# MaxMax2016/MixGAN-TTS

Hardware: AMD Instinct MI355X
Metric: denoiser steps/sec (80-mel, L=1000 frames, B=16 per GPU) (higher is better)
Workload: dtype f32

## Files before the change

mixgan-tts_amd/csrc/denoiser_common.h:

```cpp
#pragma once
#include "conv_mfma.h"
#include <cstdlib>

int mg_device_cus();
unsigned *mg_host_err_device_ptr();
unsigned mg_persist_spin_limit();
static inline bool den_persist_allowed(int NL, int tiles_per_b, int chain_cap)
{
    const char *pe = std::getenv("MG_DENOISER_PERSIST");
    return !(pe && pe[0] == '0') && NL >= 3 && tiles_per_b <= chain_cap;
}

enum DpSyncWord {
    DP_SYNC_TICKET = 0,
    DP_SYNC_ERROR = 1,
    DP_SYNC_LAUNCHES = 2,
    DP_SYNC_DONE = 3,
    DP_SYNC_TICKET_B = 16,
    DP_SYNC_WORDS = 64
};
static_assert(DP_SYNC_TICKET_B < DP_SYNC_WORDS, "every counter word lies inside the reserved block");
static_assert((int)DP_SYNC_TICKET == MG_STATUS_TICKET && (int)DP_SYNC_ERROR == MG_STATUS_ERROR && (int)DP_SYNC_LAUNCHES == MG_STATUS_LAUNCHES &&
              (int)DP_SYNC_DONE == MG_STATUS_DONE && MG_STATUS_DONE + 1 == MG_STATUS_WORDS, "one contiguous copy");

struct DenLayout {
    size_t freq, in_w, in_b, mlp0, mlp2, skip_w, skip_b, out_w, out_b, layers, layer_stride;
    size_t l_wc, l_w3, l_wo, l_bc, l_b3, l_bo, l_wd, l_wp;
    size_t bw, in_wT, skip_wT, out_wT, wc_allT, blayers, blayer_stride;
    size_t bl_w3T, bl_woT;
    size_t slayers, slayer_stride, sl_wc, sl_w3, sl_wo;
    size_t in_w16, skip_w16, out_w16, p16layers, p16layer_stride, p_wc, p_w3, p_wo;
    size_t wc_all, bc_all;
    size_t jobs;
    size_t total;
};

static inline DenLayout den_layout(const mg_denoiser_dims *d, int flags)
{
    const int with_backward = flags & MG_DEN_BACKWARD;
    const int C = d->channels, H = d->cond_channels, M = d->mel_bins, NL = d->n_layers;
    DenLayout o;
    size_t p = 0;
    auto take = [&](size_t n) {
        size_t at = p;
        p += mg_align_up(n, 64);
        return at;
    };
    o.freq = take(C / 2);
    o.in_w = take(mg_conv_packed_floats(C, M, 1, MG_PACK_PLAIN));
    o.in_b = take(C);
    o.mlp0 = take((size_t)4 * C * C);
    o.mlp2 = take((size_t)4 * C * C);
    o.skip_w = take(mg_conv_packed_floats(C, C, 1, MG_PACK_PLAIN));
    o.skip_b = take(C);
    o.out_w = take(mg_conv_packed_floats(M, C, 1, MG_PACK_PLAIN));
    o.out_b = take(M);
    o.layers = p;
    size_t q = 0;
    auto ltake = [&](size_t n) {
        size_t at = q;
        q += mg_align_up(n, 64);
        return at;
    };
    o.l_wc = ltake(mg_conv_packed_floats(C, H, 1, MG_PACK_PLAIN));
    o.l_w3 = ltake(mg_conv_packed_floats(2 * C, C, 3, MG_PACK_GATE));
    o.l_wo = ltake(mg_conv_packed_floats(2 * C, C, 1, MG_PACK_PLAIN));
    o.l_bc = ltake(C);
    o.l_b3 = ltake(2 * C);
    o.l_bo = ltake(2 * C);
    o.l_wd = ltake((size_t)C * C);
    o.l_wp = ltake(d->multi_speaker ? (size_t)C * H : 0);
    o.layer_stride = q;
    p += q * NL;
    o.bw = p;
    o.in_wT = o.skip_wT = o.out_wT = o.wc_allT = o.blayers = o.blayer_stride = o.bl_w3T = o.bl_woT = 0;
    if (with_backward) {
        o.in_wT = take(mg_conv_packed_floats(C, M, 1, MG_PACK_DGRAD));
        o.skip_wT = take(mg_conv_packed_floats(C, C, 1, MG_PACK_DGRAD));
        o.out_wT = take(mg_conv_packed_floats(M, C, 1, MG_PACK_DGRAD));
        o.wc_allT = take((size_t)mg_conv_mblocks(H) * ((size_t)NL * C / 8) * 256);
        o.blayers = p;
        size_t r = 0;
        auto btake = [&](size_t n) {
            size_t at = r;
            r += mg_align_up(n, 64);
            return at;
        };
        o.bl_w3T = btake(mg_conv_packed_floats(2 * C, C, 3, MG_PACK_DGRAD));
        o.bl_woT = btake(mg_conv_packed_floats(2 * C, C, 1, MG_PACK_DGRAD));
        o.blayer_stride = r;
        p += r * NL;
    }
    o.slayers = o.slayer_stride = o.sl_wc = o.sl_w3 = o.sl_wo = 0;
    if (flags & MG_DEN_SPLIT) {
        o.slayers = p;
        size_t r = 0;
        auto stake = [&](size_t n) {
            size_t at = r;
            r += mg_align_up(n, 64);
            return at;
        };
        o.sl_wc = stake((size_t)(C / 32) * (H / 16) * 512);
        o.sl_w3 = stake((size_t)(2 * C / 32) * (3 * C / 16) * 512);
        o.sl_wo = stake((size_t)(2 * C / 32) * (C / 16) * 512);
        o.slayer_stride = r;
        p += r * NL;
    }
    o.in_w16 = o.skip_w16 = o.out_w16 = o.p16layers = o.p16layer_stride = o.p_wc = o.p_w3 = o.p_wo = 0;
    o.wc_all = o.bc_all = 0;
    if (flags & MG_DEN_P16) {
        o.in_w16 = take(mg_conv_packed_floats(C, M, 1, MG_PACK_PLAIN16));
        o.skip_w16 = take(mg_conv_packed_floats(C, C, 1, MG_PACK_PLAIN16));
        o.out_w16 = take(mg_conv_packed_floats(M, C, 1, MG_PACK_PLAIN16));
        o.p16layers = p;
        size_t r = 0;
        auto ptake = [&](size_t n) {
            size_t at = r;
            r += mg_align_up(n, 64);
            return at;
        };
        o.p_wc = ptake(mg_conv_packed_floats(C, H, 1, MG_PACK_PLAIN16));
        o.p_w3 = ptake(mg_conv_packed_floats(2 * C, C, 3, MG_PACK_GATE16));
        o.p_wo = ptake(mg_conv_packed_floats(2 * C, C, 1, MG_PACK_PLAIN16));
        o.p16layer_stride = r;
        p += r * NL;
        o.wc_all = take((size_t)NL * mg_conv_packed_floats(C, H, 1, MG_PACK_PLAIN));
        o.bc_all = take((size_t)NL * C);
    }
    p = mg_align_up(p, 64);
    o.jobs = p;
    p += 768 * 96 / 4;
    o.total = p;
    return o;
}

static inline int den_check(const mg_denoiser_dims *d)
{
    if (!d) return MG_ERR_ARG;
    if (d->n_layers <= 0 || d->n_layers > 256 || d->channels <= 0 || d->channels % 64 || d->cond_channels <= 0 ||
        d->cond_channels % 32 || d->mel_bins <= 0)
        return MG_ERR_SHAPE;
    return MG_OK;
}

struct DenWs {
    size_t emb, h1pre, h1, s, dvec, hvec, x, skip, y, x0, h, g, sig, tnh, conds, total;
    size_t act_stride;
    size_t sync, gran;
    size_t team;
};

static inline size_t den_persist_tiles(int B, int L) { return (size_t)B * ((L + 15) / 16); }

static inline DenWs den_ws(const mg_denoiser_dims *d, int B, int L, int save)
{
    const size_t C = d->channels, NL = d->n_layers;
    const size_t act = mg_align_up((size_t)B * C * L, 64);
    DenWs w;
    size_t p = 0;
    auto take = [&](size_t n) {
        size_t at = p;
        p += mg_align_up(n, 64);
        return at;
    };
    w.emb = take(B * C);
    w.h1pre = take(B * 4 * C);
    w.h1 = take(B * 4 * C);
    w.s = take(B * C);
    w.dvec = take(NL * B * C);
    w.hvec = d->multi_speaker ? take(NL * B * C) : w.dvec;
    w.x = take(act);
    w.skip = take(act);
    w.y = take(act);
    w.x0 = save ? take(act) : w.x;
    w.act_stride = save ? act : 0;
    const size_t nact = save ? NL : 1;
    w.h = take(act * nact);
    w.g = take(act * nact);
    w.sig = save ? take(act * nact) : 0;
    w.tnh = save ? take(act * nact) : 0;
    w.conds = take(act);
    w.sync = take(DP_SYNC_WORDS);
    w.gran = take(2 * den_persist_tiles(B, L) * 2 * C * 2);
    w.team = take(den_persist_tiles(B, L) <= 128 && C == 256 ? 2 * den_persist_tiles(B, L) * 256 * (18 + 16) * 2 : 0);
    w.total = p;
    return w;
}

struct DenBws {
    size_t dout, dz_all, dx_all, dh_all, dy, dx0, scratch, dd_all, dhv_all, ds, dm, da, btop, bbot, total;
    size_t sync, gran;
};

static inline DenBws den_bws(const mg_denoiser_dims *d, int B, int L)
{
    const size_t C = d->channels, NL = d->n_layers, H = d->cond_channels, M = d->mel_bins;
    const size_t act = mg_align_up((size_t)B * C * L, 64);
    DenBws w;
    size_t p = 0;
    auto take = [&](size_t n) {
        size_t at = p;
        p += mg_align_up(n, 64);
        return at;
    };
    w.dout = take(2 * act);
    w.dz_all = take(2 * NL * act);
    w.dx_all = take((NL + 1) * act);
    w.dh_all = take(NL * act);
    w.dy = take(act);
    w.dx0 = take(act);
    size_t sc = 0;
    const int c = (int)C, h = (int)H, m = (int)M, nl = (int)NL;
    const int shapes[6][3] = {{2 * c, c, 3}, {2 * c, c, 1}, {nl * c, h, 1}, {c, m, 1}, {c, c, 1}, {m, c, 1}};
    for (const auto &sh : shapes) {
        const size_t need = mg_conv1d_wgrad_scratch_floats(sh[0], sh[1], sh[2]);
        if (need > sc) sc = need;
    }
    {
        const size_t g3 = mg_conv1d_wgrad_grouped_scratch_floats(2 * c, c, 3, nl);
        const size_t go = mg_conv1d_wgrad_grouped_scratch_floats(c, c, 1, nl);
        if (g3 > sc) sc = g3;
        if (go > sc) sc = go;
    }
    w.scratch = take(sc);
    w.btop = take((size_t)NL * C);
    w.bbot = take(C);
    w.dd_all = take(NL * B * C);
    w.dhv_all = take(NL * B * C);
    w.ds = take(B * C);
    w.dm = take(B * 4 * C);
    w.da = take(B * 4 * C);
    w.sync = take(DP_SYNC_WORDS);
    w.gran = take(2 * den_persist_tiles(B, L) * 2 * (2 * C) * 2);
    w.total = p;
    return w;
}

static __global__ void step_embed_kernel(const int64_t *__restrict__ t, const float *__restrict__ freq,
                                  float *__restrict__ emb, int B, int C)
{
    const int half = C / 2;
    const int idx = blockIdx.x * blockDim.x + threadIdx.x;
    if (idx >= B * half) return;
    const int b = idx / half, i = idx - b * half;
    const double ang = (double)((float)t[b] * freq[i]);
    emb[(size_t)b * C + i] = (float)sin(ang);
    emb[(size_t)b * C + half + i] = (float)cos(ang);
}

__device__ __forceinline__ float mg_softplus(float v) { return v > 20.f ? v : log1pf(expf(v)); }

template <int BC>
__global__ __launch_bounds__(256) void small_linear_kernel(const float *__restrict__ W, long w_zs,
                                                           const float *__restrict__ in, float *__restrict__ out,
                                                           long out_zs, const float *__restrict__ add, long add_zs,
                                                           float *__restrict__ pre, int B, int N, int K, int mish,
                                                           int in_rows)
{
    const int lane = threadIdx.x & 63;
    const int j = blockIdx.x * 4 + (threadIdx.x >> 6);
    const int b0 = blockIdx.y * BC;
    const int z = blockIdx.z;
    if (j >= N) return;
    const float *w = W + (size_t)z * w_zs + (size_t)j * K;
    float acc[BC];
#pragma unroll
    for (int b = 0; b < BC; ++b) acc[b] = 0.f;
    if ((K & 255) == 0) {
        for (int i = lane * 4; i < K; i += 256) {
            const f32x4 wv = *reinterpret_cast<const f32x4 *>(w + i);
            f32x4 xv[BC];
#pragma unroll
            for (int b = 0; b < BC; ++b)
                xv[b] = *reinterpret_cast<const f32x4 *>(in + (size_t)(min(b0 + b, B - 1) % in_rows) * K + i);
#pragma unroll
            for (int b = 0; b < BC; ++b) {
                float t = acc[b];
                t = fmaf(wv[0], xv[b][0], t);
                t = fmaf(wv[1], xv[b][1], t);
                t = fmaf(wv[2], xv[b][2], t);
                t = fmaf(wv[3], xv[b][3], t);
                acc[b] = t;
            }
        }
    } else {
        for (int i = lane; i < K; i += 64) {
            const float wv = w[i];
#pragma unroll
            for (int b = 0; b < BC; ++b)
                if (b0 + b < B) acc[b] = fmaf(wv, in[(size_t)((b0 + b) % in_rows) * K + i], acc[b]);
        }
    }
#pragma unroll
    for (int b = 0; b < BC; ++b) {
        float v = acc[b];
#pragma unroll
        for (int o = 32; o > 0; o >>= 1) v += __shfl_xor(v, o, 64);
        if (lane == 0 && b0 + b < B) {
            if (pre) pre[(size_t)(b0 + b) * N + j] = v;
            if (mish) v = v * tanhf(mg_softplus(v));
            const size_t o = (size_t)z * out_zs + (size_t)(b0 + b) * N + j;
            if (add) v += add[(size_t)z * add_zs + (size_t)(b0 + b) * N + j];
            out[o] = v;
        }
    }
}

static inline int small_linear(const float *W, long w_zs, const float *in, float *out, long out_zs, const float *add,
                               long add_zs, float *pre, int B, int N, int K, int Z, int mish, hipStream_t st,
                               int in_rows = 0)
{
    constexpr int BC = 8;
    dim3 grid(mg_cdiv(N, 4), mg_cdiv(B, BC), Z);
    hipLaunchKernelGGL(small_linear_kernel<BC>, grid, dim3(256), 0, st, W, w_zs, in, out, out_zs, add, add_zs, pre, B, N,
                       K, mish, in_rows > 0 ? in_rows : B);
    MG_LAUNCH_CHECK();
    return MG_OK;
}

static __global__ void small_outer_kernel(const float *__restrict__ a, long a_zs, long a_bs, const float *__restrict__ c,
                                   float *__restrict__ out, int Z, int B, int N, int K)
{
    const size_t n = (size_t)Z * N * K;
    for (size_t idx = (size_t)blockIdx.x * blockDim.x + threadIdx.x; idx < n; idx += (size_t)gridDim.x * blockDim.x) {
        const int j = (int)(idx % K);
        const int i = (int)((idx / K) % N);
        const int z = (int)(idx / ((size_t)K * N));
        float s = 0.f;
        for (int b = 0; b < B; ++b) s = fmaf(a[(size_t)z * a_zs + (size_t)b * a_bs + i], c[(size_t)b * K + j], s);
        out[idx] = s;
    }
}

static __global__ __launch_bounds__(256) void small_linear_t_kernel(const float *__restrict__ W, long w_zs,
                                                                    const float *__restrict__ a, long a_zs, long a_bs,
                                                                    float *__restrict__ out, int Z, int B, int N, int K)
{
    __shared__ float red[4][64];
    const int lane = threadIdx.x & 63, wave = threadIdx.x >> 6;
    const int j = blockIdx.x * 64 + lane;
    const int b = blockIdx.y, z = blockIdx.z;
    const float *w = W + (size_t)z * w_zs + min(j, K - 1);
    const float *av = a + (size_t)z * a_zs + (size_t)b * a_bs;
    const int per = (N + 3) / 4;
    const int i0 = wave * per, i1 = min(N, i0 + per);
    float s = 0.f;
#pragma unroll 8
    for (int i = i0; i < i1; ++i) s = fmaf(w[(size_t)i * K], av[i], s);
    red[wave][lane] = s;
    __syncthreads();
    if (wave == 0 && j < K) {
        const float t = red[0][lane] + red[1][lane] + red[2][lane] + red[3][lane];
        if (Z > 1) atomicAdd(out + (size_t)b * K + j, t);
        else out[(size_t)b * K + j] = t;
    }
}

static __global__ void mish_bwd_kernel(const float *__restrict__ dm, const float *__restrict__ x, float *__restrict__ da, int n)
{
    const int i = blockIdx.x * blockDim.x + threadIdx.x;
    if (i >= n) return;
    const float v = x[i];
    const float ts = tanhf(mg_softplus(v));
    const float sg = 1.f / (1.f + expf(-v));
    da[i] = dm[i] * (ts + v * (1.f - ts * ts) * sg);
}

static __global__ void scale_mask_kernel(const float *__restrict__ in, long in_bs, const float *__restrict__ mask,
                                  float *__restrict__ out, float alpha, int CL, size_t n)
{
    for (size_t i = (size_t)blockIdx.x * blockDim.x + threadIdx.x; i < n; i += (size_t)gridDim.x * blockDim.x) {
        const size_t b = i / CL;
        const size_t r = i - b * CL;
        out[i] = mask[i] > 0.f ? alpha * in[b * in_bs + r] : 0.f;
    }
}
```

mixgan-tts_amd/csrc/denoiser_persist.h:

```cpp
#pragma once
#include "common.h"
#include "denoiser_common.h"
#include "resblock_fused.h"

#define DP_SPIN_LIMIT (1u << 21)
#define DP_F_ROLES 1
#define DP_F_WITHHOLD 2

typedef unsigned long long dp_u64;
typedef __attribute__((address_space(1))) dp_u64 dp_gu64;
typedef __attribute__((address_space(1))) unsigned dp_gu32;
typedef __attribute__((address_space(1))) const char dp_gcchar;
typedef __attribute__((address_space(1))) const f32x4 dp_gcf32x4;

struct PersistArgs {
    const float *x_t;
    const float *cond;
    const float *cproj;
    float *cproj_out;
    const float *in_w, *in_b;
    const float *layers;
    size_t layer_stride, l_wc, l_w3, l_wo, l_bc, l_b3, l_bo;
    const float *p16layers;
    size_t p16layer_stride, p_wc, p_w3, p_wo;
    const float *skip_w, *skip_b, *out_w, *out_b;
    const float *hvec, *dvec;
    int vec_rows;
    float *out;
    const int64_t *t;
    const float *coef1, *coef2, *logvar;
    const float *noise;
    unsigned long long seed;
    unsigned long long noise_stream;
    float *x0_out;
    dp_u64 *gran;
    dp_u64 *team;
    unsigned *sync;
    unsigned *host_err;
    unsigned spin_limit;
    float *x0_save, *y_save, *skip_save;
    float *h_save, *g_save, *sig_save, *tnh_save;
    size_t act_stride;
    unsigned long long *dbg;
    int dbg_wave;
    int B, L, M, NL, tiles_per_b, post, clip, n_steps;
    int flags;
    float rsNL;
    int b_split;
    const float *x_t2, *hvec2, *dvec2, *cond2;
    float *out2;
};

struct DpIterK1 {
    static constexpr int N = 8, KW = 1;
    static __device__ __forceinline__ int chunk(int it) { return it; }
    static __device__ __forceinline__ int tap(int) { return 0; }
};
struct DpIterHead {
    static constexpr int N = 3, KW = 1;
    static __device__ __forceinline__ int chunk(int it) { return it; }
    static __device__ __forceinline__ int tap(int) { return 0; }
};
struct DpIterCentre {
    static constexpr int N = 8, KW = 3;
    static __device__ __forceinline__ int chunk(int it) { return it; }
    static __device__ __forceinline__ int tap(int) { return 1; }
};
struct DpIterOuter {
    static constexpr int N = 16, KW = 3;
    static __device__ __forceinline__ int chunk(int it) { return it >> 1; }
    static __device__ __forceinline__ int tap(int it) { return (it & 1) * 2; }
};

__device__ __forceinline__ int dp_pos(int ch) { return ((ch & 1) << 2) | ((ch >> 1) & 3); }
template <int NTC>
__device__ __forceinline__ int dp_at(int ch, int col) { return (((ch >> 3) * NTC + col) << 3) + dp_pos(ch); }

#ifndef DP_DIST_BIG
#define DP_DIST_BIG 3
#endif
template <int NMB, int NNB, int NTC, class IT, int DIST, bool SBASE>
__device__ __forceinline__ void dp_mfma_loop_at(f32x16 (&acc)[NMB][NNB], const f32x4 *const (&ap)[NMB], unsigned loff,
                                                const float *__restrict__ tile)
{
    static_assert(DIST >= 1 && DIST <= 3, "ring of 4 slots");
    f32x4 ring[4][NMB];
    f32x4 bb[2][NNB];
    dp_gcchar *ub[NMB];
    if (SBASE) {
#pragma unroll
        for (int i = 0; i < NMB; ++i) {
            const unsigned long long v = reinterpret_cast<unsigned long long>(ap[i]);
            const unsigned lo = __builtin_amdgcn_readfirstlane((unsigned)v), hi = __builtin_amdgcn_readfirstlane((unsigned)(v >> 32));
            ub[i] = (dp_gcchar *)(((unsigned long long)hi << 32) | lo);
        }
    }
    auto sbase = [&](int i, int qb) {
        dp_gcchar *p = ub[i] + (size_t)qb * 1024;
        asm volatile("" : "+s"(p));
        return p;
    };
    if (SBASE) asm volatile("" : "+v"(loff));
    auto wload = [&](int i, int qb, int d) -> f32x4 {
        if (SBASE) return *(dp_gcf32x4 *)(ub[i] + (size_t)qb * 1024 + loff + d * 1024);
        return ap[i][(size_t)(qb + d) * 64];
    };
    auto qbase = [](int it) { return (IT::chunk(it) * IT::KW + IT::tap(it)) * 4; };
    auto boff = [](int it) { return IT::chunk(it) * (4 * NTC * 8) + IT::tap(it) * 8; };
    {
        const int q0 = qbase(0);
#pragma unroll
        for (int s = 0; s < DIST; ++s)
#pragma unroll
            for (int i = 0; i < NMB; ++i) ring[s][i] = wload(i, q0, s);
        const float *T0 = tile + boff(0);
#pragma unroll
        for (int j = 0; j < NNB; ++j) bb[0][j] = *reinterpret_cast<const f32x4 *>(T0 + 32 * 8 * j);
    }
#pragma unroll 1
    for (int it = 0; it < IT::N; ++it) {
        const int itn = it + 1 < IT::N ? it + 1 : IT::N - 1;
        const int qc = qbase(it), qn = qbase(itn);
        const float *Tc = tile + boff(it), *Tn = tile + boff(itn);
        dp_gcchar *bc[NMB], *bn[NMB];
        if (SBASE) {
            asm volatile("" : "+v"(loff));
#pragma unroll
            for (int i = 0; i < NMB; ++i) {
                bc[i] = sbase(i, qc);
                bn[i] = sbase(i, qn);
            }
        }
#pragma unroll
        for (int u = 0; u < 4; ++u) {
#pragma unroll
            for (int i = 0; i < NMB; ++i) {
                constexpr int LIM = 4 - DIST;
                const int d = u < LIM ? u + DIST : u - LIM;
                if (SBASE) ring[(u + DIST) & 3][i] = *(dp_gcf32x4 *)((u < LIM ? bc[i] : bn[i]) + loff + d * 1024);
                else ring[(u + DIST) & 3][i] = wload(i, u < LIM ? qc : qn, d);
            }
            {
                const float *Tx = u < 3 ? Tc + (u + 1) * (NTC * 8) : Tn;
#pragma unroll
                for (int j = 0; j < NNB; ++j) bb[(u + 1) & 1][j] = *reinterpret_cast<const f32x4 *>(Tx + 32 * 8 * j);
            }
            __builtin_amdgcn_sched_barrier(0);
#pragma unroll
            for (int e = 0; e < 4; ++e) {
#pragma unroll
                for (int i = 0; i < NMB; ++i)
#pragma unroll
                    for (int j = 0; j < NNB; ++j)
                        acc[i][j] = __builtin_amdgcn_mfma_f32_32x32x2f32(ring[u][i][e], bb[u & 1][j][e], acc[i][j], 0, 0, 0);
                if (NMB * NNB < 4) __builtin_amdgcn_sched_barrier(0);
            }
            __builtin_amdgcn_sched_barrier(0);
        }
    }
}
template <int NMB, int NNB, int NTC, class IT, int DIST = (NMB * NNB >= 4 ? DP_DIST_BIG : 3)>
__device__ __forceinline__ void dp_mfma_loop(f32x16 (&acc)[NMB][NNB], const f32x4 *const (&ap)[NMB], const float *__restrict__ tile)
{
    dp_mfma_loop_at<NMB, NNB, NTC, IT, DIST, false>(acc, ap, 0u, tile);
}
template <int NMB, int NNB, int NTC, class IT, int DIST = (NMB * NNB >= 4 ? DP_DIST_BIG : 3)>
__device__ __forceinline__ void dp_mfma_loop_sbase(f32x16 (&acc)[NMB][NNB], const f32x4 *const (&ap)[NMB], unsigned loff,
                                             const float *__restrict__ tile)
{
    dp_mfma_loop_at<NMB, NNB, NTC, IT, DIST, true>(acc, ap, loff, tile);
}

template <int NTC, class F>
__device__ __forceinline__ void dp_store_block(float *T, int ch0, int col, int hh, F val)
{
#pragma unroll
    for (int q = 0; q < 4; ++q) {
        float *base = T + ((((ch0 >> 3) + q) * NTC + col) << 3);
        const f32x2 lo = {val(4 * q + 0), val(4 * q + 2)}, hi = {val(4 * q + 1), val(4 * q + 3)};
        *reinterpret_cast<f32x2 *>(base + 2 * hh) = lo;
        *reinterpret_cast<f32x2 *>(base + 4 + 2 * hh) = hi;
    }
}

__device__ __forceinline__ void dp_philox(unsigned long long seed, unsigned long long offset, unsigned long long idx,
                                          unsigned (&r)[4])
{
    unsigned c0 = (unsigned)idx, c1 = (unsigned)(idx >> 32), c2 = (unsigned)offset, c3 = (unsigned)(offset >> 32);
    unsigned k0 = (unsigned)seed, k1 = (unsigned)(seed >> 32);
#pragma unroll
    for (int i = 0; i < 10; ++i) {
        const unsigned long long p0 = (unsigned long long)0xD2511F53u * c0, p1 = (unsigned long long)0xCD9E8D57u * c2;
        const unsigned n0 = (unsigned)(p1 >> 32) ^ c1 ^ k0, n1 = (unsigned)p1, n2 = (unsigned)(p0 >> 32) ^ c3 ^ k1,
                       n3 = (unsigned)p0;
        c0 = n0; c1 = n1; c2 = n2; c3 = n3;
        k0 += 0x9E3779B9u;
        k1 += 0xBB67AE85u;
    }
    r[0] = c0; r[1] = c1; r[2] = c2; r[3] = c3;
}

__device__ __forceinline__ float dp_normal(unsigned long long seed, unsigned long long offset, unsigned long long idx)
{
    unsigned r[4];
    dp_philox(seed, offset, idx, r);
    const float u1 = ((float)r[0] + 1.0f) * 2.3283064365386963e-10f;
    const float u2 = (float)r[1] * 2.3283064365386963e-10f;
    return sqrtf(-2.0f * __logf(u1)) * __cosf(6.283185307179586f * u2);
}

#define DP_RLX_AGENT __ATOMIC_RELAXED, __HIP_MEMORY_SCOPE_AGENT

__device__ __forceinline__ void dp_fail(unsigned *sync, unsigned *host_err, unsigned code)
{
    __hip_atomic_store(sync + DP_SYNC_ERROR, code, DP_RLX_AGENT);
    if (host_err) __hip_atomic_store(host_err, code, __ATOMIC_RELAXED, __HIP_MEMORY_SCOPE_SYSTEM);
    __builtin_amdgcn_fence(__ATOMIC_RELEASE, "agent");
}
__device__ __forceinline__ bool dp_failed(unsigned *sync)
{
    __builtin_amdgcn_fence(__ATOMIC_ACQUIRE, "agent");
    return __hip_atomic_load(sync + DP_SYNC_ERROR, DP_RLX_AGENT) != 0u;
}
__device__ __forceinline__ void dp_take_ticket(int tid, unsigned *sync, unsigned &s_ticket, unsigned &s_launch, unsigned &s_dead)
{
    if (tid == 0) {
        s_ticket = __hip_atomic_fetch_add(sync + DP_SYNC_TICKET, 1u, DP_RLX_AGENT);
        s_launch = __hip_atomic_load(sync + DP_SYNC_LAUNCHES, DP_RLX_AGENT);
        s_dead = 0u;
    }
}
template <bool QUEUE_B>
__device__ __forceinline__ void dp_retire(int tid, unsigned *sync, int n_slots)
{
    if (tid == 0) {
        const unsigned done = __hip_atomic_fetch_add(sync + DP_SYNC_DONE, 1u, DP_RLX_AGENT);
        if (done == (unsigned)n_slots - 1u) {
            __hip_atomic_store(sync + DP_SYNC_DONE, 0u, DP_RLX_AGENT);
            __hip_atomic_store(sync + DP_SYNC_TICKET, 0u, DP_RLX_AGENT);
            if (QUEUE_B) __hip_atomic_store(sync + DP_SYNC_TICKET_B, 0u, DP_RLX_AGENT);
            __hip_atomic_fetch_add(sync + DP_SYNC_LAUNCHES, 1u, DP_RLX_AGENT);
        }
    }
}
#define DP_EPOCH(launch_no, NL, step) ((launch_no) * ((unsigned)(NL) + 1u) + (unsigned)(step) + 1u)

struct DpPosterior { float c1, c2, sg; };
__device__ __forceinline__ DpPosterior dp_posterior_at(const PersistArgs &a, int b)
{
    long tb = (long)a.t[b];
    tb = tb < 0 ? 0 : (tb >= a.n_steps ? a.n_steps - 1 : tb);
    const float c1 = a.coef1[tb], c2 = a.coef2[tb];
    const float sg = tb == 0 ? 0.f : __expf(0.5f * a.logvar[tb]);
    return {c1, c2, sg};
}
__device__ __forceinline__ float dp_clip_x0(float x0, int clip)
{
    if (clip) x0 = fminf(fmaxf(x0, -1.f), 1.f);
    return x0;
}
__device__ __forceinline__ float dp_posterior(const DpPosterior &p, float x0, float xt, float nz) { return fmaf(p.sg, nz, fmaf(p.c1, x0, p.c2 * xt)); }
#define DP_STAMP(k) do { if (TIMING && tid == 64 * a.dbg_wave) a.dbg[((size_t)tile * (a.NL + 2) + stamp_row) * 12 + (k)] = clock64(); } while (0)

template <int NT, int RW>
__device__ __forceinline__ void dp_cproj_fetch(const float *cp, float *cl, int w, int lane, int l0, int L)
{
    constexpr int LPR = NT / 4;
    constexpr int RPI = 64 / LPR;
    const int rsub = lane / LPR, c4 = lane - rsub * LPR;
    unsigned off = (unsigned)(((RW * w + rsub) * L + min(l0 + 4 * c4, L - 4)) * 4);
    asm volatile("" : "+v"(off));
    float *dst = cl + (size_t)RW * w * NT;
    const unsigned at = (unsigned)(size_t)(__attribute__((address_space(3))) void *)dst;
#pragma unroll
    for (int it = 0; it < RW / RPI; ++it) {
        const float *gi = cp + (size_t)it * RPI * L;
        const unsigned m = __builtin_amdgcn_readfirstlane(at + (unsigned)(it * RPI * NT * 4));
        asm volatile("s_mov_b32 m0, %0\n\ts_nop 0\n\tglobal_load_lds_dwordx4 %1, %2" : : "s"(m), "v"(off), "s"(gi) : "memory");
    }
}

template <int NT, bool VEC4, bool TIMING = false, bool SAVE = false, int NWV = NT / 8, int CPM = 0, bool SOLO = false>
__global__ __launch_bounds__(NWV * 64, ((NT == 64 && NWV == 4) || SOLO) ? 1 : 2) void denoiser_persist_kernel(PersistArgs a)
{
    static_assert(!SOLO || (NT == 32 && NWV == 4), "SOLO is the one-per-CU build of the 4-wave 32-frame form");
    static_assert(!(CPM && SAVE), "the saving forward computes its projections and keeps none");
    constexpr bool READP = CPM == 2, WRITEP = CPM == 1;
#ifndef DP_DIST_SOLO
#define DP_DIST_SOLO 2
#endif
    constexpr int DBIG = ((NT == 64 && NWV == 4) || SOLO) ? DP_DIST_SOLO : DP_DIST_BIG;
#ifndef DP_ONEPASS_WHEN
#define DP_ONEPASS_WHEN (MB == 2 && ((NT == 64 && NWV == 4) || SOLO))
#endif
    static_assert((NT == 32 && (NWV == 4 || NWV == 8)) || (NT == 64 && (NWV == 8 || NWV == 4)),
                  "tile widths: 32 frames (4 waves, two workgroups per CU; or 8 waves, one per CU) or 64 (8 waves, one)");
    constexpr int NTHR = NWV * 64, NW = NWV;
    constexpr bool TWO_PER_CU = NT == 32 && NWV == 4;
    constexpr int MB = 8 / NW;
    constexpr bool ONEPASS = DP_ONEPASS_WHEN;
    constexpr int NNB = NT / 32;
    constexpr int NC = NT, NH = NT + 2;
    __shared__ __attribute__((aligned(16))) float lds[RB_C * (NC + NH)];
    __shared__ unsigned s_tile, s_dead, s_launch;
    float *condT = lds;
    float *hT = lds + RB_C * NC;

    const int tid = threadIdx.x, lane = tid & 63, w = tid >> 6;
    const int hh = lane >> 5, c32 = lane & 31;
    const int L = a.L;
    const int wu = __builtin_amdgcn_readfirstlane(w);
    const unsigned loff = (unsigned)lane * 16u;

    const int n_tiles = a.tiles_per_b * a.B;
    const unsigned hw_id = __builtin_amdgcn_s_getreg((31 << 11) | 4);
    const int role = (TWO_PER_CU && (a.flags & DP_F_ROLES)) ? (int)(hw_id & 1u) : 0;
    if (tid == 0) {
        const int nA = (TWO_PER_CU && (a.flags & DP_F_ROLES)) ? (a.B / 2) * a.tiles_per_b : n_tiles;
        const int n_mine = role == 0 ? nA : n_tiles - nA;
        unsigned tk = __hip_atomic_fetch_add(a.sync + (role ? DP_SYNC_TICKET_B : DP_SYNC_TICKET), 1u, DP_RLX_AGENT);
        int tl;
        if ((int)tk < n_mine) tl = (role == 0 ? 0 : nA) + (int)tk;
        else {
            tk = __hip_atomic_fetch_add(a.sync + (role ? DP_SYNC_TICKET : DP_SYNC_TICKET_B), 1u, DP_RLX_AGENT);
            tl = (role == 0 ? nA : 0) + (int)tk;
        }
        s_tile = (unsigned)tl;
        s_launch = __hip_atomic_load(a.sync + DP_SYNC_LAUNCHES, DP_RLX_AGENT);
        s_dead = 0u;
    }
    __syncthreads();
    const int tile = min((int)s_tile, n_tiles - 1);
    const unsigned launch_no = s_launch;
    const int bg = tile / a.tiles_per_b, jt = tile - bg * a.tiles_per_b;
    const bool second = a.b_split > 0 && bg >= a.b_split;
    const int b = second ? bg - a.b_split : bg;
    const int Bp = a.b_split > 0 ? (second ? a.B - a.b_split : a.b_split) : a.B;
    const bool do_save = SAVE && (a.b_split == 0 || second);
    const float *const x_in = second ? a.x_t2 : a.x_t;
    float *const x_out = second ? a.out2 : a.out;
    const int l0 = jt * NT;
    const bool has_left = jt > 0, has_right = jt + 1 < a.tiles_per_b;
    int stamp_row = 0;
    DP_STAMP(0);
    if (TIMING && tid == 0) {
        a.dbg[((size_t)tile * (a.NL + 2)) * 12 + 2] = hw_id;
        a.dbg[((size_t)tile * (a.NL + 2)) * 12 + 3] = __builtin_amdgcn_s_getreg((31 << 11) | 20);
    }

    {
        const float *cb = (second ? a.cond2 : a.cond) + (size_t)b * RB_C * L;
        if (READP) {
            if (VEC4) dp_cproj_fetch<NT, 32 * MB>(a.cproj + (size_t)b * a.NL * RB_C * L, lds, w, lane, l0, L);
        } else if (VEC4) {
#pragma unroll
            for (int k = 0; k < 64 * NT / NTHR; ++k) {
                const int idx = tid + k * NTHR;
                const int row = idx / (NT / 4), c4 = idx - row * (NT / 4);
                const int f0 = l0 + 4 * c4;
                const bool ok = f0 < L;
                const f32x4 v = *reinterpret_cast<const f32x4 *>(cb + (size_t)row * L + min(f0, L - 4));
#pragma unroll
                for (int e = 0; e < 4; ++e) condT[dp_at<NC>(row, 4 * c4 + e)] = ok ? v[e] : 0.f;
            }
        } else {
#pragma unroll
            for (int k = 0; k < 256 * NT / NTHR; ++k) {
                const int idx = tid + k * NTHR;
                const int row = idx / NT, cc = idx - row * NT;
                const int f = l0 + cc;
                const float v = cb[(size_t)row * L + min(f, L - 1)];
                condT[dp_at<NC>(row, cc)] = f < L ? v : 0.f;
            }
        }
        const float *xb = x_in + (size_t)b * a.M * L;
#pragma unroll
        for (int k = 0; k < 96 * NT / NTHR; ++k) {
            const int idx = tid + k * NTHR;
            const int row = idx / NT, c = idx - row * NT;
            const int f = l0 + c;
            const float v = xb[(size_t)min(row, a.M - 1) * L + min(f, L - 1)];
            hT[dp_at<NH>(row, c)] = (row < a.M && f < L) ? v : 0.f;
        }
    }

    f32x16 st[2 * MB][NNB];
    const int rbase = 32 * MB * w;
    auto row_of = [&](int i, int r) { return rbase + 32 * i + 8 * (r >> 2) + 4 * hh + (r & 3); };
#pragma unroll
    for (int i = 0; i < MB; ++i)
#pragma unroll
        for (int j = 0; j < NNB; ++j)
#pragma unroll
            for (int r = 0; r < 16; ++r) {
                st[i][j][r] = a.in_b[row_of(i, r)];
                st[MB + i][j][r] = 0.f;
            }
    __syncthreads();
    {
        f32x16 acc[MB][NNB];
        const f32x4 *ap[MB];
#pragma unroll
        for (int i = 0; i < MB; ++i) {
            ap[i] = reinterpret_cast<const f32x4 *>(a.in_w) + (size_t)(MB * wu + i) * 12 * 64;
#pragma unroll
            for (int j = 0; j < NNB; ++j) acc[i][j] = st[i][j];
        }
        dp_mfma_loop_sbase<MB, NNB, NH, DpIterHead>(acc, ap, loff, hT + c32 * 8 + hh * 4);
#pragma unroll
        for (int i = 0; i < MB; ++i)
#pragma unroll
            for (int j = 0; j < NNB; ++j)
#pragma unroll
                for (int r = 0; r < 16; ++r) st[i][j][r] = fmaxf(acc[i][j][r], 0.f);
    }
    DP_STAMP(1);
    bool fvalid[NNB];
    const size_t bbase = (size_t)b * RB_C * L;
    auto save_block = [&](float *dst, int ch0, int j, auto val) {
        const int f = l0 + 32 * j + c32;
        if (f < L) {
#pragma unroll
            for (int r = 0; r < 16; ++r) dst[bbase + (size_t)(ch0 + 8 * (r >> 2) + 4 * hh + (r & 3)) * L + f] = val(r);
        }
    };
#pragma unroll
    for (int j = 0; j < NNB; ++j) fvalid[j] = l0 + 32 * j + c32 < L;
    if (SAVE && do_save) {
#pragma unroll
        for (int i = 0; i < MB; ++i)
#pragma unroll
            for (int j = 0; j < NNB; ++j) save_block(a.x0_save, rbase + 32 * i, j, [&](int r) { return st[i][j][r]; });
    }
    dp_gu64 *const gran = (dp_gu64 *)a.gran;

    for (int l = 0; l < a.NL; ++l) {
        const float *lp = a.layers + (size_t)l * a.layer_stride;
        const size_t vrows = a.vec_rows ? (size_t)a.vec_rows : (size_t)Bp;
        const float *hv = (second ? a.hvec2 : a.hvec) + ((size_t)l * vrows + b) * RB_C;
        const float *dv = (second ? a.dvec2 : a.dvec) + ((size_t)l * vrows + b) * RB_C;
        const unsigned epoch = DP_EPOCH(launch_no, a.NL, l);
        const int par = l & 1;
        stamp_row = l + 1;
        DP_STAMP(0);

        f32x16 acc1[MB][NNB];
        if (READP && VEC4) {
            asm volatile("s_waitcnt vmcnt(0)" ::: "memory");
#pragma unroll
            for (int i = 0; i < MB; ++i)
#pragma unroll
                for (int j = 0; j < NNB; ++j)
#pragma unroll
                    for (int r = 0; r < 16; ++r) acc1[i][j][r] = lds[row_of(i, r) * NT + 32 * j + c32];
        } else if (READP) {
            const float *cp = a.cproj + ((size_t)b * a.NL + l) * RB_C * L;
#pragma unroll
            for (int i = 0; i < MB; ++i)
#pragma unroll
                for (int j = 0; j < NNB; ++j) {
                    unsigned lo = (unsigned)((rbase + 4 * hh) * L + min(l0 + 32 * j + c32, L - 1));
                    asm volatile("" : "+v"(lo));
#pragma unroll
                    for (int r = 0; r < 16; ++r) acc1[i][j][r] = cp[lo + (unsigned)((32 * i + 8 * (r >> 2) + (r & 3)) * L)];
                }
        } else {
#pragma unroll
            for (int i = 0; i < MB; ++i)
#pragma unroll
                for (int j = 0; j < NNB; ++j)
#pragma unroll
                    for (int r = 0; r < 16; ++r) acc1[i][j][r] = lp[a.l_bc + row_of(i, r)];
            const f32x4 *wc = reinterpret_cast<const f32x4 *>(lp + a.l_wc);
            const f32x4 *ap[MB];
#pragma unroll
            for (int i = 0; i < MB; ++i) ap[i] = wc + (size_t)(MB * wu + i) * 32 * 64;
            dp_mfma_loop_sbase<MB, NNB, NC, DpIterK1, (MB * NNB >= 4 ? DBIG : 3)>(acc1, ap, loff, condT + c32 * 8 + hh * 4);
            if (WRITEP) {
                float *co = a.cproj_out + ((size_t)b * a.NL + l) * RB_C * L;
                unsigned lo = (unsigned)((rbase + 4 * hh) * L + l0 + c32);
                asm volatile("" : "+v"(lo));
#pragma unroll
                for (int i = 0; i < MB; ++i)
#pragma unroll
                    for (int j = 0; j < NNB; ++j)
                        if (l0 + 32 * j + c32 < L) {
#pragma unroll
                            for (int r = 0; r < 16; ++r)
                                co[lo + (unsigned)((32 * i + 8 * (r >> 2) + (r & 3)) * L + 32 * j)] = acc1[i][j][r];
                        }
            }
        }
#pragma unroll
        for (int i = 0; i < MB; ++i)
#pragma unroll
            for (int j = 0; j < NNB; ++j)
#pragma unroll
                for (int r = 0; r < 16; ++r) acc1[i][j][r] += st[i][j][r] + hv[row_of(i, r)];
        DP_STAMP(1);
        f32x16 acc2[MB][2][NNB];
#pragma unroll
        for (int p = 0; p < MB; ++p)
#pragma unroll
            for (int r = 0; r < 16; ++r) {
                const int ch = row_of(p, r);
                const float bg = lp[a.l_b3 + ch], bf = lp[a.l_b3 + RB_C + ch];
#pragma unroll
                for (int j = 0; j < NNB; ++j) {
                    acc2[p][0][j][r] = bg;
                    acc2[p][1][j][r] = bf;
                }
            }
        __syncthreads();
        DP_STAMP(2);
#pragma unroll
        for (int i = 0; i < MB; ++i)
#pragma unroll
            for (int j = 0; j < NNB; ++j)
            {
                dp_store_block<NH>(hT, rbase + 32 * i, 1 + 32 * j + c32, hh,
                                   [&](int r) { return fvalid[j] ? acc1[i][j][r] : 0.f; });
                if (SAVE && do_save) save_block(a.h_save + (size_t)l * a.act_stride, rbase + 32 * i, j, [&](int r) { return acc1[i][j][r]; });
            }
        if (READP && VEC4 && l + 1 < a.NL)
            dp_cproj_fetch<NT, 32 * MB>(a.cproj + ((size_t)b * a.NL + l + 1) * RB_C * L, lds, w, lane, l0, L);
        __syncthreads();
        DP_STAMP(3);

        if (w < 2) {
            bool go = w == 0 ? has_left : has_right;
            if ((a.flags & DP_F_WITHHOLD) && w == 0 && jt == 1) go = false;
            if (go) {
                const int dst_tile = w == 0 ? tile - 1 : tile + 1;
                const int col = w == 0 ? 1 : NT;
                dp_gu64 *g = gran + (((size_t)par * n_tiles + dst_tile) * 2 + (w == 0 ? 1 : 0)) * RB_C;
#pragma unroll
                for (int k = 0; k < 4; ++k) {
                    const int row = lane + 64 * k;
                    const dp_u64 v = ((dp_u64)epoch << 32) | (dp_u64)__float_as_uint(hT[dp_at<NH>(row, col)]);
                    __hip_atomic_store(g + row, v, DP_RLX_AGENT);
                }
            }
        }

        const f32x4 *w3 = reinterpret_cast<const f32x4 *>(lp + a.l_w3);
        const f32x4 *ap2[MB][2];
#pragma unroll
        for (int p = 0; p < MB; ++p) {
            ap2[p][0] = w3 + (size_t)(2 * (MB * wu + p)) * 96 * 64;
            ap2[p][1] = w3 + (size_t)(2 * (MB * wu + p) + 1) * 96 * 64;
        }
        if (ONEPASS) {
            dp_mfma_loop_sbase<2 * MB, NNB, NH, DpIterCentre, DBIG>(reinterpret_cast<f32x16 (&)[2 * MB][NNB]>(acc2),
                                                              reinterpret_cast<const f32x4 *const (&)[2 * MB]>(ap2), loff,
                                                              hT + c32 * 8 + hh * 4);
        } else {
#pragma unroll
            for (int p = 0; p < MB; ++p)
                dp_mfma_loop_sbase<2, NNB, NH, DpIterCentre, (2 * NNB >= 4 ? DBIG : 3)>(acc2[p], ap2[p], loff, hT + c32 * 8 + hh * 4);
        }
        DP_STAMP(4);

        if (w < 2) {
            const bool from = w == 0 ? has_left : has_right;
            const int col = w == 0 ? 0 : NT + 1;
            unsigned v[4] = {0u, 0u, 0u, 0u};
            if (from && s_dead == 0u) {
                dp_gu64 *g = gran + (((size_t)par * n_tiles + tile) * 2 + w) * RB_C;
                unsigned spins = 0;
                for (;;) {
                    bool ok = true;
#pragma unroll
                    for (int k = 0; k < 4; ++k) {
                        const dp_u64 x = __hip_atomic_load(g + lane + 64 * k, DP_RLX_AGENT);
                        v[k] = (unsigned)x;
                        ok &= (unsigned)(x >> 32) == epoch;
                    }
                    if (__all(ok)) break;
                    if (++spins > a.spin_limit) {
                        if (lane == 0) {
                            dp_fail(a.sync, a.host_err, 1u + (unsigned)l);
                            s_dead = 1u;
                        }
                        break;
                    }
                    __builtin_amdgcn_s_sleep(8);
                }
            }
#pragma unroll
            for (int k = 0; k < 4; ++k) hT[dp_at<NH>(lane + 64 * k, col)] = from ? __uint_as_float(v[k]) : 0.f;
        }
        DP_STAMP(5);
        __syncthreads();
        DP_STAMP(6);

        if (ONEPASS) {
            dp_mfma_loop_sbase<2 * MB, NNB, NH, DpIterOuter, DBIG>(reinterpret_cast<f32x16 (&)[2 * MB][NNB]>(acc2),
                                                             reinterpret_cast<const f32x4 *const (&)[2 * MB]>(ap2), loff,
                                                             hT + c32 * 8 + hh * 4);
        } else {
#pragma unroll
            for (int p = 0; p < MB; ++p)
                dp_mfma_loop_sbase<2, NNB, NH, DpIterOuter, (2 * NNB >= 4 ? DBIG : 3)>(acc2[p], ap2[p], loff, hT + c32 * 8 + hh * 4);
        }
        DP_STAMP(7);
        __syncthreads();
        DP_STAMP(8);
#pragma unroll
        for (int p = 0; p < MB; ++p)
#pragma unroll
            for (int j = 0; j < NNB; ++j)
            {
                if (SAVE && do_save) {
#pragma unroll
                    for (int r = 0; r < 16; ++r) {
                        acc2[p][0][j][r] = mg_sigmoid(acc2[p][0][j][r]);
                        acc2[p][1][j][r] = mg_tanh(acc2[p][1][j][r]);
                    }
                    const size_t lo = (size_t)l * a.act_stride;
                    save_block(a.sig_save + lo, rbase + 32 * p, j, [&](int r) { return acc2[p][0][j][r]; });
                    save_block(a.tnh_save + lo, rbase + 32 * p, j, [&](int r) { return acc2[p][1][j][r]; });
                    save_block(a.g_save + lo, rbase + 32 * p, j, [&](int r) { return acc2[p][0][j][r] * acc2[p][1][j][r]; });
                    dp_store_block<NH>(hT, rbase + 32 * p, 32 * j + c32, hh, [&](int r) { return acc2[p][0][j][r] * acc2[p][1][j][r]; });
                } else {
                    dp_store_block<NH>(hT, rbase + 32 * p, 32 * j + c32, hh,
                                       [&](int r) { return mg_sigmoid(acc2[p][0][j][r]) * mg_tanh(acc2[p][1][j][r]); });
                }
            }
#pragma unroll
        for (int i = 0; i < MB; ++i)
#pragma unroll
            for (int j = 0; j < NNB; ++j)
#pragma unroll
                for (int r = 0; r < 16; ++r) {
                    const int row = row_of(i, r);
                    st[i][j][r] += lp[a.l_bo + row] + dv[row];
                    st[MB + i][j][r] += lp[a.l_bo + RB_C + row];
                }
        DP_STAMP(9);
        __syncthreads();
        DP_STAMP(10);

        {
            const f32x4 *wo = reinterpret_cast<const f32x4 *>(lp + a.l_wo);
            const f32x4 *ap[2 * MB];
#pragma unroll
            for (int i = 0; i < MB; ++i) {
                ap[i] = wo + (size_t)(MB * wu + i) * 32 * 64;
                ap[MB + i] = wo + (size_t)(8 + MB * wu + i) * 32 * 64;
            }
            dp_mfma_loop_sbase<2 * MB, NNB, NH, DpIterK1, (2 * MB * NNB >= 4 ? DBIG : 3)>(st, ap, loff, hT + c32 * 8 + hh * 4);
        }
        DP_STAMP(11);
#pragma unroll
        for (int i = 0; i < MB; ++i)
#pragma unroll
            for (int j = 0; j < NNB; ++j)
#pragma unroll
                for (int r = 0; r < 16; ++r) st[i][j][r] *= 0.70710678118654752440f;
    }

    stamp_row = a.NL + 1;
    DP_STAMP(0);
    __syncthreads();
#pragma unroll
    for (int i = 0; i < MB; ++i)
#pragma unroll
        for (int j = 0; j < NNB; ++j)
            {
                dp_store_block<NH>(hT, rbase + 32 * i, 32 * j + c32, hh, [&](int r) { return st[MB + i][j][r] * a.rsNL; });
                if (SAVE && do_save) save_block(a.skip_save, rbase + 32 * i, j, [&](int r) { return st[MB + i][j][r]; });
            }
    __syncthreads();
    {
        f32x16 acc[MB][NNB];
        const f32x4 *ap[MB];
#pragma unroll
        for (int i = 0; i < MB; ++i) {
            ap[i] = reinterpret_cast<const f32x4 *>(a.skip_w) + (size_t)(MB * wu + i) * 32 * 64;
#pragma unroll
            for (int j = 0; j < NNB; ++j)
#pragma unroll
                for (int r = 0; r < 16; ++r) acc[i][j][r] = a.skip_b[row_of(i, r)];
        }
        dp_mfma_loop_sbase<MB, NNB, NH, DpIterK1>(acc, ap, loff, hT + c32 * 8 + hh * 4);
#pragma unroll
        for (int i = 0; i < MB; ++i)
#pragma unroll
            for (int j = 0; j < NNB; ++j)
            {
                dp_store_block<NC>(condT, rbase + 32 * i, 32 * j + c32, hh, [&](int r) { return fmaxf(acc[i][j][r], 0.f); });
                if (SAVE && do_save) save_block(a.y_save, rbase + 32 * i, j, [&](int r) { return fmaxf(acc[i][j][r], 0.f); });
            }
    }
    __syncthreads();
    const int mblocks = (a.M + 31) / 32;
    for (int task = wu; task < mblocks * NNB; task += NW) {
        const int mb = task / NNB, nb = task - mb * NNB;
        f32x16 o[1][1];
#pragma unroll
        for (int r = 0; r < 16; ++r) {
            const int row = 32 * mb + 8 * (r >> 2) + 4 * hh + (r & 3);
            o[0][0][r] = row < a.M ? a.out_b[row] : 0.f;
        }
        const f32x4 *const ap[1] = {reinterpret_cast<const f32x4 *>(a.out_w) + (size_t)mb * 32 * 64};
        dp_mfma_loop_sbase<1, 1, NC, DpIterK1>(o, ap, loff, condT + (32 * nb + c32) * 8 + hh * 4);
        const int f = l0 + 32 * nb + c32;
        const size_t bo = (size_t)b * a.M * L;
        const bool bad = dp_failed(a.sync);
        const float poison = __builtin_nanf("");
        if (!a.post) {
#pragma unroll
            for (int r = 0; r < 16; ++r) {
                const int row = 32 * mb + 8 * (r >> 2) + 4 * hh + (r & 3);
                if (row < a.M && f < L) x_out[bo + (size_t)row * L + f] = bad ? poison : o[0][0][r];
            }
        } else {
            const DpPosterior ps = dp_posterior_at(a, b);
            const unsigned long long seed = a.seed, off = (a.noise_stream << 32) | (unsigned long long)launch_no;
            const int fc = min(f, L - 1);
            float xt[16], nz[16];
#pragma unroll
            for (int r = 0; r < 16; ++r) {
                const int row = min(32 * mb + 8 * (r >> 2) + 4 * hh + (r & 3), a.M - 1);
                const size_t e = bo + (size_t)row * L + fc;
                xt[r] = a.x_t[e];
                nz[r] = a.noise ? a.noise[e] : dp_normal(seed, off, e);
            }
#pragma unroll
            for (int r = 0; r < 16; ++r) {
                const int row = 32 * mb + 8 * (r >> 2) + 4 * hh + (r & 3);
                if (row < a.M && f < L) {
                    const size_t e = bo + (size_t)row * L + f;
                    float x0 = o[0][0][r];
                    if (a.x0_out) a.x0_out[e] = x0;
                    x0 = dp_clip_x0(x0, a.clip);
                    a.out[e] = bad ? poison : dp_posterior(ps, x0, xt[r], nz[r]);
                }
            }
        }
    }
    DP_STAMP(1);
    dp_retire<true>(tid, a.sync, n_tiles);
}
```

Baseline: 383.2.

## Fuse conv3 centre/outer MFMA loops with halo prefetch; grid-stride small linear

The centre and outer tap passes of the dilated conv become one loop split at a seam. The halo atomic loads are issued early, inside the last centre iteration, so the neighbour exchange latency overlaps MFMA work and the ring pipeline no longer drains between the two loops. small_linear now uses a grid-stride loop capped at 8 workgroups per CU, keeps weights in registers across batch chunks when K is a multiple of 256 and at most 1024, and has lanes write outputs in parallel. A readfirstlane fix for the scalar global pointer in the LDS load is also included.

```diff
diff --git a/mixgan-tts_amd/csrc/denoiser_common.h b/mixgan-tts_amd/csrc/denoiser_common.h
--- a/mixgan-tts_amd/csrc/denoiser_common.h
+++ b/mixgan-tts_amd/csrc/denoiser_common.h
@@ -1,5 +1,6 @@
 #pragma once
 #include "conv_mfma.h"
+#include <algorithm>
 #include <cstdlib>
 
 int mg_device_cus();
@@ -250,58 +251,70 @@
 
 __device__ __forceinline__ float mg_softplus(float v) { return v > 20.f ? v : log1pf(expf(v)); }
 
-template <int BC>
+template <int BC, int KV>
 __global__ __launch_bounds__(256) void small_linear_kernel(const float *__restrict__ W, long w_zs,
                                                            const float *__restrict__ in, float *__restrict__ out,
                                                            long out_zs, const float *__restrict__ add, long add_zs,
-                                                           float *__restrict__ pre, int B, int N, int K, int mish,
+                                                           float *__restrict__ pre, int B, int N, int K, int Z, int mish,
                                                            int in_rows)
 {
     const int lane = threadIdx.x & 63;
-    const int j = blockIdx.x * 4 + (threadIdx.x >> 6);
-    const int b0 = blockIdx.y * BC;
-    const int z = blockIdx.z;
-    if (j >= N) return;
-    const float *w = W + (size_t)z * w_zs + (size_t)j * K;
-    float acc[BC];
-#pragma unroll
-    for (int b = 0; b < BC; ++b) acc[b] = 0.f;
-    if ((K & 255) == 0) {
-        for (int i = lane * 4; i < K; i += 256) {
-            const f32x4 wv = *reinterpret_cast<const f32x4 *>(w + i);
-            f32x4 xv[BC];
-#pragma unroll
-            for (int b = 0; b < BC; ++b)
-                xv[b] = *reinterpret_cast<const f32x4 *>(in + (size_t)(min(b0 + b, B - 1) % in_rows) * K + i);
+    const int rows = Z * N;
+    for (int row = blockIdx.x * 4 + (threadIdx.x >> 6); row < rows; row += gridDim.x * 4) {
+        const int z = row / N, j = row - z * N;
+        const float *w = W + (size_t)z * w_zs + (size_t)j * K;
+        f32x4 wk[KV > 0 ? KV : 1];
+        if (KV > 0) {
+#pragma unroll
+            for (int m = 0; m < KV; ++m) wk[m] = *reinterpret_cast<const f32x4 *>(w + lane * 4 + 256 * m);
+        }
+        for (int b0 = blockIdx.y * BC; b0 < B; b0 += gridDim.y * BC) {
+            float acc[BC];
+#pragma unroll
+            for (int b = 0; b < BC; ++b) acc[b] = 0.f;
+            auto chain = [&](const f32x4 &wv, int i) {
+                f32x4 xv[BC];
+#pragma unroll
+                for (int b = 0; b < BC; ++b)
+                    xv[b] = *reinterpret_cast<const f32x4 *>(in + (size_t)(min(b0 + b, B - 1) % in_rows) * K + i);
+#pragma unroll
+                for (int b = 0; b < BC; ++b) {
+                    float t = acc[b];
+                    t = fmaf(wv[0], xv[b][0], t);
+                    t = fmaf(wv[1], xv[b][1], t);
+                    t = fmaf(wv[2], xv[b][2], t);
+                    t = fmaf(wv[3], xv[b][3], t);
+                    acc[b] = t;
+                }
+            };
+            if (KV > 0) {
+#pragma unroll
+                for (int m = 0; m < KV; ++m) chain(wk[m], lane * 4 + 256 * m);
+            } else if ((K & 255) == 0) {
+                for (int i = lane * 4; i < K; i += 256) chain(*reinterpret_cast<const f32x4 *>(w + i), i);
+            } else {
+                for (int i = lane; i < K; i += 64) {
+                    const float wv = w[i];
+#pragma unroll
+                    for (int b = 0; b < BC; ++b)
+                        if (b0 + b < B) acc[b] = fmaf(wv, in[(size_t)((b0 + b) % in_rows) * K + i], acc[b]);
+                }
+            }
+            float v = 0.f;
 #pragma unroll
             for (int b = 0; b < BC; ++b) {
-                float t = acc[b];
-                t = fmaf(wv[0], xv[b][0], t);
-                t = fmaf(wv[1], xv[b][1], t);
-                t = fmaf(wv[2], xv[b][2], t);
-                t = fmaf(wv[3], xv[b][3], t);
-                acc[b] = t;
+                float s = acc[b];
+#pragma unroll
+                for (int o = 32; o > 0; o >>= 1) s += __shfl_xor(s, o, 64);
+                if (lane == b) v = s;
             }
-        }
-    } else {
-        for (int i = lane; i < K; i += 64) {
-            const float wv = w[i];
-#pragma unroll
-            for (int b = 0; b < BC; ++b)
-                if (b0 + b < B) acc[b] = fmaf(wv, in[(size_t)((b0 + b) % in_rows) * K + i], acc[b]);
-        }
-    }
-#pragma unroll
-    for (int b = 0; b < BC; ++b) {
-        float v = acc[b];
-#pragma unroll
-        for (int o = 32; o > 0; o >>= 1) v += __shfl_xor(v, o, 64);
-        if (lane == 0 && b0 + b < B) {
-            if (pre) pre[(size_t)(b0 + b) * N + j] = v;
-            if (mish) v = v * tanhf(mg_softplus(v));
-            const size_t o = (size_t)z * out_zs + (size_t)(b0 + b) * N + j;
-            if (add) v += add[(size_t)z * add_zs + (size_t)(b0 + b) * N + j];
-            out[o] = v;
+            if (lane < BC && b0 + lane < B) {
+                const size_t at = (size_t)(b0 + lane) * N + j;
+                if (pre) pre[at] = v;
+                if (mish) v = v * tanhf(mg_softplus(v));
+                if (add) v += add[(size_t)z * add_zs + at];
+                out[(size_t)z * out_zs + at] = v;
+            }
         }
     }
 }
@@ -311,9 +324,14 @@
                                int in_rows = 0)
 {
     constexpr int BC = 8;
-    dim3 grid(mg_cdiv(N, 4), mg_cdiv(B, BC), Z);
-    hipLaunchKernelGGL(small_linear_kernel<BC>, grid, dim3(256), 0, st, W, w_zs, in, out, out_zs, add, add_zs, pre, B, N,
-                       K, mish, in_rows > 0 ? in_rows : B);
+    const int WGS = 8 * mg_device_cus();
+    const int gx = std::min(mg_cdiv(Z * N, 4), WGS), chunks = mg_cdiv(B, BC);
+    dim3 grid(gx, std::max(1, std::min(chunks, WGS / gx)), 1);
+    const int kv = (K & 255) == 0 && K <= 1024 ? K / 256 : 0;
+    auto *kern = kv == 1 ? small_linear_kernel<BC, 1> : kv == 2 ? small_linear_kernel<BC, 2> : kv == 3 ? small_linear_kernel<BC, 3>
+               : kv == 4 ? small_linear_kernel<BC, 4> : small_linear_kernel<BC, 0>;
+    hipLaunchKernelGGL(kern, grid, dim3(256), 0, st, W, w_zs, in, out, out_zs, add, add_zs, pre, B, N, K, Z, mish,
+                       in_rows > 0 ? in_rows : B);
     MG_LAUNCH_CHECK();
     return MG_OK;
 }
diff --git a/mixgan-tts_amd/csrc/denoiser_persist.h b/mixgan-tts_amd/csrc/denoiser_persist.h
--- a/mixgan-tts_amd/csrc/denoiser_persist.h
+++ b/mixgan-tts_amd/csrc/denoiser_persist.h
@@ -71,6 +71,14 @@
     static __device__ __forceinline__ int chunk(int it) { return it >> 1; }
     static __device__ __forceinline__ int tap(int it) { return (it & 1) * 2; }
 };
+struct DpIterConv3 {
+    static constexpr int N = 24, KW = 3, SPLIT = DpIterCentre::N;
+    static __device__ __forceinline__ int chunk(int it) { return it < SPLIT ? it : (it - SPLIT) >> 1; }
+    static __device__ __forceinline__ int tap(int it) { return it < SPLIT ? 1 : ((it - SPLIT) & 1) * 2; }
+};
+struct DpNoHook {
+    __device__ __forceinline__ void operator()() const {}
+};
 
 __device__ __forceinline__ int dp_pos(int ch) { return ((ch & 1) << 2) | ((ch >> 1) & 3); }
 template <int NTC>
@@ -79,10 +87,11 @@
 #ifndef DP_DIST_BIG
 #define DP_DIST_BIG 3
 #endif
-template <int NMB, int NNB, int NTC, class IT, int DIST, bool SBASE>
+template <int NMB, int NNB, int NTC, class IT, int DIST, bool SBASE, int SPLIT = 0, class PRE = DpNoHook, class MID = DpNoHook>
 __device__ __forceinline__ void dp_mfma_loop_at(f32x16 (&acc)[NMB][NNB], const f32x4 *const (&ap)[NMB], unsigned loff,
-                                                const float *__restrict__ tile)
-{
+                                                const float *__restrict__ tile, PRE pre = PRE(), MID mid = MID())
+{
+    static_assert(SPLIT >= 0 && SPLIT < IT::N, "the seam lies inside the loop");
     static_assert(DIST >= 1 && DIST <= 3, "ring of 4 slots");
     f32x4 ring[4][NMB];
     f32x4 bb[2][NNB];
@@ -117,8 +126,7 @@
 #pragma unroll
         for (int j = 0; j < NNB; ++j) bb[0][j] = *reinterpret_cast<const f32x4 *>(T0 + 32 * 8 * j);
     }
-#pragma unroll 1
-    for (int it = 0; it < IT::N; ++it) {
+    auto kiter = [&](int it, auto hook) __attribute__((always_inline)) {
         const int itn = it + 1 < IT::N ? it + 1 : IT::N - 1;
         const int qc = qbase(it), qn = qbase(itn);
         const float *Tc = tile + boff(it), *Tn = tile + boff(itn);
@@ -145,6 +153,7 @@
 #pragma unroll
                 for (int j = 0; j < NNB; ++j) bb[(u + 1) & 1][j] = *reinterpret_cast<const f32x4 *>(Tx + 32 * 8 * j);
             }
+            if (u == 3) hook();
             __builtin_amdgcn_sched_barrier(0);
 #pragma unroll
             for (int e = 0; e < 4; ++e) {
@@ -157,6 +166,22 @@
             }
             __builtin_amdgcn_sched_barrier(0);
         }
+    };
+    if constexpr (SPLIT == 0) {
+#pragma unroll 1
+        for (int it = 0; it < IT::N; ++it) kiter(it, DpNoHook());
+    } else {
+#pragma unroll 1
+        for (int it = 0; it < SPLIT - 1; ++it) kiter(it, DpNoHook());
+        kiter(SPLIT - 1, pre);
+        mid();
+        {
+            const float *Ts = tile + boff(SPLIT);
+#pragma unroll
+            for (int j = 0; j < NNB; ++j) bb[0][j] = *reinterpret_cast<const f32x4 *>(Ts + 32 * 8 * j);
+        }
+#pragma unroll 1
+        for (int it = SPLIT; it < IT::N; ++it) kiter(it, DpNoHook());
     }
 }
 template <int NMB, int NNB, int NTC, class IT, int DIST = (NMB * NNB >= 4 ? DP_DIST_BIG : 3)>
@@ -169,6 +194,12 @@
                                              const float *__restrict__ tile)
 {
     dp_mfma_loop_at<NMB, NNB, NTC, IT, DIST, true>(acc, ap, loff, tile);
+}
+template <int NMB, int NNB, int NTC, class IT, int DIST, class PRE, class MID>
+__device__ __forceinline__ void dp_mfma_loop_sbase_split(f32x16 (&acc)[NMB][NNB], const f32x4 *const (&ap)[NMB], unsigned loff,
+                                                         const float *__restrict__ tile, PRE pre, MID mid)
+{
+    dp_mfma_loop_at<NMB, NNB, NTC, IT, DIST, true, IT::SPLIT, PRE, MID>(acc, ap, loff, tile, pre, mid);
 }
 
 template <int NTC, class F>
@@ -274,7 +305,9 @@
     const unsigned at = (unsigned)(size_t)(__attribute__((address_space(3))) void *)dst;
 #pragma unroll
     for (int it = 0; it < RW / RPI; ++it) {
-        const float *gi = cp + (size_t)it * RPI * L;
+        const unsigned long long gv = reinterpret_cast<unsigned long long>(cp + (size_t)it * RPI * L);
+        const unsigned glo = __builtin_amdgcn_readfirstlane((unsigned)gv), ghi = __builtin_amdgcn_readfirstlane((unsigned)(gv >> 32));
+        const float *gi = reinterpret_cast<const float *>(((unsigned long long)ghi << 32) | glo);
         const unsigned m = __builtin_amdgcn_readfirstlane(at + (unsigned)(it * RPI * NT * 4));
         asm volatile("s_mov_b32 m0, %0\n\ts_nop 0\n\tglobal_load_lds_dwordx4 %1, %2" : : "s"(m), "v"(off), "s"(gi) : "memory");
     }
@@ -550,55 +583,67 @@
             ap2[p][0] = w3 + (size_t)(2 * (MB * wu + p)) * 96 * 64;
             ap2[p][1] = w3 + (size_t)(2 * (MB * wu + p) + 1) * 96 * 64;
         }
+        dp_u64 gpre[4];
+        auto halo_prefetch = [&]() {
+            const bool from = w < 2 && (w == 0 ? has_left : has_right);
+            dp_gu64 *g = gran + (((size_t)par * n_tiles + tile) * 2 + (w & 1)) * RB_C;
+#pragma unroll
+            for (int k = 0; k < 4; ++k) gpre[k] = from ? __hip_atomic_load(g + lane + 64 * k, DP_RLX_AGENT) : (dp_u64)0;
+        };
+        auto halo_receive = [&](bool prefetched) {
+            DP_STAMP(4);
+            if (w < 2) {
+                const bool from = w == 0 ? has_left : has_right;
+                const int col = w == 0 ? 0 : NT + 1;
+                unsigned v[4] = {0u, 0u, 0u, 0u};
+                if (from && s_dead == 0u) {
+                    dp_gu64 *g = gran + (((size_t)par * n_tiles + tile) * 2 + w) * RB_C;
+                    bool have = prefetched;
+                    if (prefetched) {
+#pragma unroll
+                        for (int k = 0; k < 4; ++k) {
+                            v[k] = (unsigned)gpre[k];
+                            have &= (unsigned)(gpre[k] >> 32) == epoch;
+                        }
+                        have = __all(have);
+                    }
+                    unsigned spins = 0;
+                    while (!have) {
+                        bool ok = true;
+#pragma unroll
+                        for (int k = 0; k < 4; ++k) {
+                            const dp_u64 x = __hip_atomic_load(g + lane + 64 * k, DP_RLX_AGENT);
+                            v[k] = (unsigned)x;
+                            ok &= (unsigned)(x >> 32) == epoch;
+                        }
+                        if (__all(ok)) break;
+                        if (++spins > a.spin_limit) {
+                            if (lane == 0) {
+                                dp_fail(a.sync, a.host_err, 1u + (unsigned)l);
+                                s_dead = 1u;
+                            }
+                            break;
+                        }
+                        __builtin_amdgcn_s_sleep(8);
+                    }
+                }
+#pragma unroll
+                for (int k = 0; k < 4; ++k) hT[dp_at<NH>(lane + 64 * k, col)] = from ? __uint_as_float(v[k]) : 0.f;
+            }
+            DP_STAMP(5);
+            __syncthreads();
+            DP_STAMP(6);
+        };
         if (ONEPASS) {
-            dp_mfma_loop_sbase<2 * MB, NNB, NH, DpIterCentre, DBIG>(reinterpret_cast<f32x16 (&)[2 * MB][NNB]>(acc2),
-                                                              reinterpret_cast<const f32x4 *const (&)[2 * MB]>(ap2), loff,
-                                                              hT + c32 * 8 + hh * 4);
+            dp_mfma_loop_sbase_split<2 * MB, NNB, NH, DpIterConv3, DBIG>(reinterpret_cast<f32x16 (&)[2 * MB][NNB]>(acc2),
+                                                                         reinterpret_cast<const f32x4 *const (&)[2 * MB]>(ap2), loff,
+                                                                         hT + c32 * 8 + hh * 4, halo_prefetch,
+                                                                         [&]() { halo_receive(true); });
         } else {
 #pragma unroll
             for (int p = 0; p < MB; ++p)
                 dp_mfma_loop_sbase<2, NNB, NH, DpIterCentre, (2 * NNB >= 4 ? DBIG : 3)>(acc2[p], ap2[p], loff, hT + c32 * 8 + hh * 4);
-        }
-        DP_STAMP(4);
-
-        if (w < 2) {
-            const bool from = w == 0 ? has_left : has_right;
-            const int col = w == 0 ? 0 : NT + 1;
-            unsigned v[4] = {0u, 0u, 0u, 0u};
-            if (from && s_dead == 0u) {
-                dp_gu64 *g = gran + (((size_t)par * n_tiles + tile) * 2 + w) * RB_C;
-                unsigned spins = 0;
-                for (;;) {
-                    bool ok = true;
-#pragma unroll
-                    for (int k = 0; k < 4; ++k) {
-                        const dp_u64 x = __hip_atomic_load(g + lane + 64 * k, DP_RLX_AGENT);
-                        v[k] = (unsigned)x;
-                        ok &= (unsigned)(x >> 32) == epoch;
-                    }
-                    if (__all(ok)) break;
-                    if (++spins > a.spin_limit) {
-                        if (lane == 0) {
-                            dp_fail(a.sync, a.host_err, 1u + (unsigned)l);
-                            s_dead = 1u;
-                        }
-                        break;
-                    }
-                    __builtin_amdgcn_s_sleep(8);
-                }
-            }
-#pragma unroll
-            for (int k = 0; k < 4; ++k) hT[dp_at<NH>(lane + 64 * k, col)] = from ? __uint_as_float(v[k]) : 0.f;
-        }
-        DP_STAMP(5);
-        __syncthreads();
-        DP_STAMP(6);
-
-        if (ONEPASS) {
-            dp_mfma_loop_sbase<2 * MB, NNB, NH, DpIterOuter, DBIG>(reinterpret_cast<f32x16 (&)[2 * MB][NNB]>(acc2),
-                                                             reinterpret_cast<const f32x4 *const (&)[2 * MB]>(ap2), loff,
-                                                             hT + c32 * 8 + hh * 4);
-        } else {
+            halo_receive(false);
 #pragma unroll
             for (int p = 0; p < MB; ++p)
                 dp_mfma_loop_sbase<2, NNB, NH, DpIterOuter, (2 * NNB >= 4 ? DBIG : 3)>(acc2[p], ap2[p], loff, hT + c32 * 8 + hh * 4);
```

After: 384.3 (median of 2 runs). About the same (+0.3%).
